# langtech-bsc/quantool

Measured on AMD Instinct MI355X. Metric: quantized weights/sec (GPTQ int4, Llama-3-8B, 512 calib samples), higher is better.
Workload: dtype f32

## Files before the change

quantool_amd/csrc/build.py:

```python
from __future__ import annotations

import hashlib
import os
import shutil
import subprocess
import sys
from concurrent.futures import ThreadPoolExecutor
from pathlib import Path

CSRC = Path(__file__).resolve().parent
PKG = CSRC.parent
LIB_DIR = PKG / "lib"
OBJ_DIR = CSRC / "_obj"
LIB_PATH = LIB_DIR / "libquantool_hip.so"

HIPCC_FLAGS = [
    "--offload-arch=gfx950",
    "-O3",
    "-fPIC",
    "-std=c++17",
    "-ffp-contract=off",
    "-fhip-fp32-correctly-rounded-divide-sqrt",
    "-fno-fast-math",
    "-Wall",
    "-Wno-unused-function",
    "-Rpass-analysis=kernel-resource-usage",
]

SCRATCH_OK: tuple = ()

HIPCC_FLAGS += os.environ.get("QT_EXTRA_HIPCC_FLAGS", "").split()


def _hipcc() -> str:
    for cand in (os.environ.get("HIPCC"), shutil.which("hipcc"), "/opt/rocm/bin/hipcc"):
        if cand and Path(cand).exists():
            return cand
    raise RuntimeError("hipcc not found (set HIPCC or install ROCm)")


def sources():
    return sorted(CSRC.glob("*.hip"))


def _stamp(src: Path) -> str:
    h = hashlib.sha1()
    h.update(src.read_bytes())
    for hdr in sorted(list(CSRC.glob("*.h")) + [PKG.parent / "include" / "quantool_amd.h"]):
        h.update(hdr.read_bytes())
    h.update(" ".join(HIPCC_FLAGS).encode())
    return h.hexdigest()


def _compile(src: Path) -> Path:
    obj = OBJ_DIR / (src.stem + ".o")
    stamp = OBJ_DIR / (src.stem + ".stamp")
    want = _stamp(src)
    if obj.exists() and stamp.exists() and stamp.read_text() == want:
        return obj
    cmd = [_hipcc(), *HIPCC_FLAGS, "-c", str(src), "-o", str(obj)]
    res = subprocess.run(cmd, capture_output=True, text=True)
    if res.returncode != 0:
        raise RuntimeError(f"hipcc failed for {src.name}:\n{res.stdout}\n{res.stderr}")
    rest = _resources(src, res.stderr)
    if rest.strip():
        sys.stderr.write(rest)
    stamp.write_text(want)
    return obj


def _resources(src: Path, stderr: str) -> str:
    import re

    kernels, cur, rest = [], None, []
    lines = stderr.splitlines()
    i = 0
    while i < len(lines):
        line = lines[i]
        m = re.search(r"remark:\s+(.*?) \[-Rpass-analysis=kernel-resource-usage\]", line)
        if m:
            kv = m.group(1).strip()
            if kv.startswith("Function Name:"):
                cur = {"name": kv.split(":", 1)[1].strip()}
                kernels.append(cur)
            elif cur is not None and ":" in kv:
                k, v = kv.rsplit(":", 1)
                cur[k.strip()] = v.strip()
            while i + 1 < len(lines) and re.match(r"^\s+\d* ?\|", lines[i + 1]):
                i += 1
        elif not re.match(r"^\d+ (warning|remark)s? generated", line.strip()) and "remarks generated" not in line:
            rest.append(line)
        i += 1
    rows = []
    for k in kernels:
        rows.append(f"{k['name']}\tvgpr {k.get('VGPRs', '?')}\tagpr {k.get('AGPRs', '?')}\tscratch "
                    f"{k.get('ScratchSize [bytes/lane]', '?')}\tvgpr_spill {k.get('VGPRs Spill', '?')}\tlds "
                    f"{k.get('LDS Size [bytes/block]', '?')}\twaves_per_simd {k.get('Occupancy [waves/SIMD]', '?')}")
    (OBJ_DIR / (src.stem + ".resources.txt")).write_text("\n".join(rows) + ("\n" if rows else ""))
    bad = [k["name"] for k in kernels
           if k.get("ScratchSize [bytes/lane]", "0") not in ("0", "?") and not any(ok in k["name"] for ok in SCRATCH_OK)]
    if bad:
        raise RuntimeError(f"{src.name}: kernel(s) with a private segment (scratch): {bad} -- see "
                           f"{OBJ_DIR / (src.stem + '.resources.txt')}; a by-value argument struct that is modified and "
                           "indexed at run time, or a register array indexed at run time, is the usual cause")
    return "\n".join(rest) + ("\n" if rest else "")


def audit_m0(src: Path) -> None:
    stamp = OBJ_DIR / (src.stem + ".m0audit")
    want = _stamp(src)
    if stamp.exists() and stamp.read_text() == want:
        return
    asm = OBJ_DIR / (src.stem + ".device.s")
    cmd = [_hipcc(), *[f for f in HIPCC_FLAGS if f != "-fPIC"], "--cuda-device-only", "-S", str(src), "-o", str(asm)]
    res = subprocess.run(cmd, capture_output=True, text=True)
    if res.returncode != 0:
        raise RuntimeError(f"hipcc -S failed for {src.name}:\n{res.stderr}")
    inside = False
    for n, line in enumerate(asm.read_text().splitlines(), 1):
        if ";;#ASMSTART" in line:
            inside = True
        elif ";;#ASMEND" in line:
            inside = False
        elif not inside and "m0" in line.split(";")[0].replace("_m0", ""):
            raise RuntimeError(f"{src.name}: compiler-generated use of M0 at {asm.name}:{n}: {line.strip()!r} -- "
                               "the LDS-DMA helpers must save/restore M0 again")
    audit_spills(src.name, asm.read_text())
    asm.unlink()
    stamp.write_text(want)


NO_SPILL_KERNELS = ("xtx_kernel", "xtx16_kernel", "gemm3_kernel", "sgemm_ring_kernel", "quantize_tokens_kernel",
                    "gemm_i8_kernel", "gemm_i8_ring_kernel", "gemm_i8_ring_moe_kernel", "gemm_i8_mid_kernel",
                    "gemm_i8_ring_w4_kernel", "gemm_i8_ring_w4_moe_kernel", "moe_gemm_i8_wide_kernel",
                    "moe_gemm_wq_wide_kernel")


def audit_spills(src_name: str, asm_text: str) -> None:
    name = None
    for line in asm_text.splitlines():
        t = line.strip()
        if t.startswith(".name:"):
            name = t.split(":", 1)[1].strip()
        elif name and t.startswith((".vgpr_spill_count:", ".private_segment_fixed_size:")):
            if int(t.split(":", 1)[1]) != 0 and any(k in name for k in NO_SPILL_KERNELS):
                raise RuntimeError(f"{src_name}: {name} spills ({t}) -- its schedule assumes every value stays in registers")


def build(verbose: bool = False) -> Path:
    OBJ_DIR.mkdir(exist_ok=True)
    LIB_DIR.mkdir(exist_ok=True)
    srcs = sources()
    with ThreadPoolExecutor(max_workers=min(8, len(srcs))) as ex:
        objs = list(ex.map(_compile, srcs))
    for name in ("xtx.hip", "gemm3_tn.hip", "sgemm_tn.hip", "qlinear.hip", "qlinear_ring.hip", "qlinear_ring_w4.hip"):
        audit_m0(CSRC / name)
    newest = max(o.stat().st_mtime for o in objs)
    if not LIB_PATH.exists() or LIB_PATH.stat().st_mtime < newest:
        cmd = [_hipcc(), "--offload-arch=gfx950", "-shared", "-fPIC", "-o", str(LIB_PATH), *map(str, objs)]
        res = subprocess.run(cmd, capture_output=True, text=True)
        if res.returncode != 0:
            raise RuntimeError(f"link failed:\n{res.stdout}\n{res.stderr}")
    if verbose:
        print(f"built {LIB_PATH}")
    return LIB_PATH


if __name__ == "__main__":
    build(verbose=True)
```

quantool_amd/csrc/cholesky.hip:

```cpp
#include <stdlib.h>
#include <string.h>

#include <map>
#include <tuple>
#include <vector>

#include "common.h"
#include "gemm3_tn.h"
#include "sgemm_tn.h"

namespace {

constexpr int NB = 128;
constexpr int NBO_MAX = 1024;
static int chol_block_env(const char* name) {
    const char* e = getenv(name);
    if (!e) return 0;
    int x = atoi(e) / 128 * 128;
    return x < 128 ? 128 : (x > NBO_MAX ? NBO_MAX : x);
}
struct G3Step {
    int n_items = 0, n_red = 0;
    size_t item_off = 0, red_off = 0;
};
struct CholG3Plan {
    bool any = false;
    std::vector<G3Step> fac, inv;
    char* blob = nullptr;
    size_t blob_bytes = 0;
    int max_slabs = 0;
};

static int chol_g3_min_chunks() {
    const char* on = getenv("QT_CHOL_G3");
    if (on && atoi(on) == 0) return 0;
    const char* e = getenv("QT_CHOL_G3_MIN_CHUNKS");
    const int x = e ? atoi(e) : 64;
    return x < 1 ? 1 : x;
}

static int chol_g3_target_items(int K) {
    const char* e = getenv("QT_G3_TARGET_ITEMS");
    if (e && atoi(e) > 0) return atoi(e);
    return K < 8192 ? 96 : 256;
}

static const CholG3Plan* chol_g3_plan(int K, int NBO, int NBI) {
    static std::mutex m;
    static std::map<std::tuple<int, int, int, int>, CholG3Plan*> plans;
    const int min_chunks = chol_g3_min_chunks();
    const int target_items = chol_g3_target_items(K);
    std::lock_guard<std::mutex> lock(m);
    const auto key = std::make_tuple(K, NBO, NBI, min_chunks * 1024 + target_items);
    auto it = plans.find(key);
    if (it != plans.end()) return it->second;
    CholG3Plan* pl = new CholG3Plan();
    std::vector<char> bytes;
    auto add = [&](int Tm, int Tn, int c_end, int tri) {
        G3Step st;
        if (min_chunks <= 0 || K % 8 != 0 || g3_row_chunks(Tm, Tn, c_end, tri) * G3_CHUNK_ROWS < (long)min_chunks * 128) return st;
        std::vector<G3Item> items;
        std::vector<G3Red> red;
        g3_plan_row(Tm, Tn, c_end, tri, items, red, target_items);
        st.n_items = (int)items.size();
        st.n_red = (int)red.size();
        st.item_off = qt_align_up(bytes.size(), 256);
        bytes.resize(st.item_off + items.size() * sizeof(G3Item));
        memcpy(bytes.data() + st.item_off, items.data(), items.size() * sizeof(G3Item));
        st.red_off = qt_align_up(bytes.size(), 256);
        bytes.resize(st.red_off + red.size() * sizeof(G3Red));
        if (!red.empty()) memcpy(bytes.data() + st.red_off, red.data(), red.size() * sizeof(G3Red));
        for (const G3Red& r : red) pl->max_slabs = pl->max_slabs > r.first + r.count ? pl->max_slabs : r.first + r.count;
        pl->any = true;
        return st;
    };
    for (int J0 = 0; J0 < K; J0 += NBO) {
        const int J1 = (K - J0 < NBO) ? K : J0 + NBO;
        pl->fac.push_back(J0 == 0 ? G3Step() : add((J1 - J0 + 255) / 256, (K - J0 + 255) / 256, J0 / G3_CHUNK_ROWS, 0));
    }
    for (int I0 = 0; I0 < K; I0 += NBI) {
        const int I1 = (K - I0 < NBI) ? K : I0 + NBI;
        pl->inv.push_back(I0 == 0 ? G3Step() : add((I1 - I0 + 255) / 256, (I0 + 255) / 256, I0 / G3_CHUNK_ROWS, 1));
    }
    if (pl->any) {
        pl->blob_bytes = qt_align_up(bytes.size(), 256);
        if (hipHostMalloc((void**)&pl->blob, pl->blob_bytes, hipHostMallocDefault) != hipSuccess) {
            pl->any = false;
            pl->blob = nullptr;
        } else {
            memcpy(pl->blob, bytes.data(), bytes.size());
        }
    }
    if (!pl->any) {
        pl->blob_bytes = 0;
        pl->max_slabs = 0;
        for (G3Step& st : pl->fac) st = G3Step();
        for (G3Step& st : pl->inv) st = G3Step();
    }
    plans[key] = pl;
    return pl;
}
static size_t chol_g3_ws_bytes(const CholG3Plan* pl, int K) {
    if (!pl->any) return 0;
    return 2 * qt_align_up((size_t)3 * K * K * 2, 256) + (size_t)pl->max_slabs * 256 * 256 * 4 + pl->blob_bytes + 256;
}

static const CholG3Plan* chol_blocks(int K, int& NBO, int& NBI) {
    const int eo = chol_block_env("QT_CHOL_NBO"), ei = chol_block_env("QT_CHOL_NBI");
    NBO = eo ? eo : 512;
    NBI = ei ? ei : 512;
    const CholG3Plan* pl = chol_g3_plan(K, NBO, NBI);
    if (pl->any) return pl;
    NBO = eo ? eo : 256;
    NBI = ei ? ei : 256;
    return chol_g3_plan(K, NBO, NBI);
}

constexpr int LDP = NB + 1;

constexpr int LDT = NB + 4;
constexpr int RD_STRIDE = NB * NB + 4 * 32 * 32;

#define QT_SEL4(kb, v0, v1, v2, v3) ((kb) == 0 ? (v0) : (kb) == 1 ? (v1) : (kb) == 2 ? (v2) : (v3))

constexpr int LDA = NB + 4;

__device__ __forceinline__ float readlane_f(float v, int lane) {
    return __int_as_float(__builtin_amdgcn_readlane(__float_as_int(v), lane));
}

__device__ __forceinline__ void mma32_tn(const float* A, int lda, const float* B, int ldb, f32x16& acc,
                                         int l31, int h, bool negate_a) {
#pragma unroll
    for (int kk = 0; kk < 16; ++kk) {
        float a = A[(2 * kk + h) * lda + l31];
        const float b = B[(2 * kk + h) * ldb + l31];
        if (negate_a) a = -a;
        acc = __builtin_amdgcn_mfma_f32_32x32x2f32(a, b, acc, 0, 0, 0);
    }
}

constexpr int POTF2_THREADS = 512, POTF2_WAVES = POTF2_THREADS / 64;
__global__ __launch_bounds__(POTF2_THREADS) void potf2_kernel(const float* P, int64_t ldp, int n,
                                                    float* Rout, int64_t ldr,
                                                    float* __restrict__ Rd, int32_t* info, int col0, int prio,
                                                    int64_t bsP, int64_t bsRd) {
    qt_set_chain_prio(prio);
    if (blockIdx.x) {
        P += (size_t)blockIdx.x * bsP;
        Rout += (size_t)blockIdx.x * bsP;
        Rd += (size_t)blockIdx.x * bsRd;
        info += blockIdx.x;
    }
    extern __shared__ __attribute__((aligned(16))) float sm[];
    float* As = sm;
    float* Xs = sm + NB * LDA;
    const int tid = threadIdx.x, lane = tid & 63;
    const int wave = __builtin_amdgcn_readfirstlane(tid >> 6);
    const int l31 = lane & 31, h = lane >> 5;

    if ((ldp & 3) == 0 && (n & 3) == 0 && (((uintptr_t)P) & 15) == 0) {
        constexpr int NV = NB * NB / 4 / POTF2_THREADS;
        f32x4 v[NV];
#pragma unroll
        for (int r = 0; r < NV; ++r) {
            const int e4 = tid + POTF2_THREADS * r;
            const int i = e4 >> 5, j = (e4 & 31) * 4;
            const int ic = i < n ? i : n - 1, jc = j < n ? j : n - 4;
            v[r] = *(const f32x4*)(P + (size_t)ic * ldp + jc);
        }
#pragma unroll
        for (int r = 0; r < NV; ++r) {
            const int e4 = tid + POTF2_THREADS * r;
            const int i = e4 >> 5, j = (e4 & 31) * 4;
            f32x4 x;
#pragma unroll
            for (int q = 0; q < 4; ++q) x[q] = (i < n && j + q < n) ? v[r][q] : (i == j + q ? 1.0f : 0.0f);
            *(f32x4*)(As + i * LDA + j) = x;
        }
    } else {
        for (int e = tid; e < NB * NB; e += POTF2_THREADS) {
            const int i = e / NB, j = e % NB;
            const int lo = i < j ? i : j, hi = i < j ? j : i;
            float v = (i == j) ? 1.0f : 0.0f;
            if (hi < n) v = P[(size_t)lo * ldp + hi];
            As[i * LDA + j] = v;
        }
    }
    __syncthreads();

    int bad = 0;
#pragma unroll 1
    for (int kb = 0; kb < 4; ++kb) {
        float* Akk = As + (32 * kb) * LDA + 32 * kb;
        if (wave == 0) {
            f32x16 c1, c2;
#pragma unroll
            for (int r = 0; r < 16; ++r) {
                const int i = (r & 3) + 8 * (r >> 2) + 4 * h;
                c1[r] = Akk[i * LDA + l31];
                c2[r] = (i == l31) ? 1.0f : 0.0f;
            }
#pragma unroll
            for (int c = 0; c < 32; ++c) {
                const int rc = (c & 3) + 4 * (c >> 3);
                const int hc = (c >> 2) & 1;
                float piv = readlane_f(c1[rc], c + 32 * hc);
                const bool isbad = !(piv > 0.0f);
                bad = (isbad && bad == 0 && 32 * kb + c < n) ? 32 * kb + c + 1 : bad;
                piv = isbad ? 1.0f : piv;
                float rs = __builtin_amdgcn_rsqf(piv);
                rs = rs * fmaf(-0.5f * piv * rs, rs, 1.5f);
                const bool mine = h == hc;
                const float rr = c1[rc] * rs, zz = c2[rc] * rs;
                c1[rc] = mine ? rr : c1[rc];
                c2[rc] = mine ? zz : c2[rc];
                if (c < 31) {
                    const float a = (mine && l31 > c) ? -rr : 0.0f;
                    const float b1 = (mine && l31 >= c) ? rr : 0.0f, b2 = mine ? zz : 0.0f;
                    c1 = __builtin_amdgcn_mfma_f32_32x32x2f32(a, b1, c1, 0, 0, 0);
                    c2 = __builtin_amdgcn_mfma_f32_32x32x2f32(a, b2, c2, 0, 0, 0);
                }
            }
#pragma unroll
            for (int r = 0; r < 16; ++r) {
                const int i = (r & 3) + 8 * (r >> 2) + 4 * h;
                Akk[i * LDA + l31] = (i <= l31) ? c1[r] : 0.0f;
                Xs[(kb * 32 + l31) * 32 + i] = (i >= l31) ? c2[r] : 0.0f;
            }
        }
        __syncthreads();
        if (kb == 3) break;
        for (int a = kb + 1 + wave; a < 4; a += POTF2_WAVES) {
            f32x16 acc;
#pragma unroll
            for (int r = 0; r < 16; ++r) acc[r] = 0.0f;
            float* Bt = As + (32 * kb) * LDA + 32 * a;
            mma32_tn(Xs + kb * 1024, 32, Bt, LDA, acc, l31, h, false);
#pragma unroll
            for (int r = 0; r < 16; ++r) Bt[((r & 3) + 8 * (r >> 2) + 4 * h) * LDA + l31] = acc[r];
        }
        __syncthreads();
        {
            int t = 0;
            for (int a = kb + 1; a < 4; ++a)
                for (int a2 = a; a2 < 4; ++a2, ++t) {
                    if ((t % POTF2_WAVES) != wave) continue;
                    float* Ct = As + (32 * a) * LDA + 32 * a2;
                    f32x16 acc;
#pragma unroll
                    for (int r = 0; r < 16; ++r) acc[r] = Ct[((r & 3) + 8 * (r >> 2) + 4 * h) * LDA + l31];
                    mma32_tn(As + (32 * kb) * LDA + 32 * a, LDA, As + (32 * kb) * LDA + 32 * a2, LDA, acc, l31, h,
                             true);
#pragma unroll
                    for (int r = 0; r < 16; ++r) Ct[((r & 3) + 8 * (r >> 2) + 4 * h) * LDA + l31] = acc[r];
                }
        }
        __syncthreads();
    }
    if (bad != 0 && tid == 0) atomicCAS(info, 0, col0 + bad);
    const bool vec_out = (ldr & 3) == 0 && (n & 3) == 0 && (((uintptr_t)Rout) & 15) == 0;
    for (int e4 = tid; e4 < NB * NB / 4; e4 += POTF2_THREADS) {
        const int i = e4 >> 5, j = (e4 & 31) * 4;
        f32x4 v = *(const f32x4*)(As + i * LDA + j);
#pragma unroll
        for (int q = 0; q < 4; ++q) v[q] = (j + q >= i) ? v[q] : 0.0f;
        *(f32x4*)(Rd + i * NB + j) = v;
        if (i < n && j + 3 >= i && j < n) {
            if (vec_out) {
                *(f32x4*)(Rout + (size_t)i * ldr + j) = v;
            } else {
#pragma unroll
                for (int q = 0; q < 4; ++q)
                    if (j + q >= i && j + q < n) Rout[(size_t)i * ldr + j + q] = v[q];
            }
        }
    }
    for (int e4 = tid; e4 < 4 * 32 * 32 / 4; e4 += POTF2_THREADS) *(f32x4*)(Rd + NB * NB + 4 * e4) = *(const f32x4*)(Xs + 4 * e4);
}

__global__ __launch_bounds__(256) void trsm_rt_kernel(const float* __restrict__ Rd, int n,
                                                      const float* B, int64_t ldb,
                                                      float* Z, int64_t ldz, int ncols, int prio, int64_t bsRd,
                                                      int64_t bsB) {
    qt_set_chain_prio(prio);
    if (blockIdx.y) {
        Rd += (size_t)blockIdx.y * bsRd;
        B += (size_t)blockIdx.y * bsB;
        Z += (size_t)blockIdx.y * bsB;
    }
    extern __shared__ __attribute__((aligned(16))) float Rs[];
    const int tid = threadIdx.x, lane = tid & 63, wave = tid >> 6;
    const float* D32 = Rs + NB * NB;
    const int l31 = lane & 31, h = lane >> 5;
    const int col = blockIdx.x * 128 + wave * 32 + l31;
    const bool cok = col < ncols;
    const int colc = cok ? col : ncols - 1;

    f32x16 acc[4];
#pragma unroll
    for (int a = 0; a < 4; ++a)
#pragma unroll
        for (int r = 0; r < 16; ++r) {
            const int row = 32 * a + (r & 3) + 8 * (r >> 2) + 4 * h;
            acc[a][r] = (row < n) ? B[(size_t)row * ldb + colc] : 0.0f;
        }
    {
        constexpr int NV = RD_STRIDE / 4 / 256;
        static_assert(NV * 4 * 256 == RD_STRIDE, "whole float4s per thread");
        f32x4 v[NV];
#pragma unroll
        for (int r = 0; r < NV; ++r) v[r] = ((const f32x4*)Rd)[tid + 256 * r];
#pragma unroll
        for (int r = 0; r < NV; ++r) ((f32x4*)Rs)[tid + 256 * r] = v[r];
    }
    __syncthreads();

#pragma unroll
    for (int b = 0; b < 4; ++b) {
        f32x16 zb;
#pragma unroll
        for (int r = 0; r < 16; ++r) zb[r] = 0.0f;
#pragma unroll
        for (int r = 0; r < 16; ++r) {
            const int k = (r & 3) + 8 * (r >> 2) + 4 * h;
            const float av = D32[(b * 32 + k) * 32 + l31];
            zb = __builtin_amdgcn_mfma_f32_32x32x2f32(av, acc[b][r], zb, 0, 0, 0);
        }
        acc[b] = zb;
#pragma unroll
        for (int a = b + 1; a < 4; ++a) {
#pragma unroll
            for (int r = 0; r < 16; ++r) {
                const int k = (r & 3) + 8 * (r >> 2) + 4 * h;
                const float av = -Rs[(32 * b + k) * NB + 32 * a + l31];
                acc[a] = __builtin_amdgcn_mfma_f32_32x32x2f32(av, zb[r], acc[a], 0, 0, 0);
            }
        }
    }
    if (cok) {
#pragma unroll
        for (int a = 0; a < 4; ++a)
#pragma unroll
            for (int r = 0; r < 16; ++r) {
                const int row = 32 * a + (r & 3) + 8 * (r >> 2) + 4 * h;
                if (row < n) Z[(size_t)row * ldz + col] = acc[a][r];
            }
    }
}

__global__ __launch_bounds__(128) void trinv_batched_kernel(const float* __restrict__ Rd_all, int K,
                                                            float* __restrict__ Dinv_all,
                                                            float* __restrict__ Y, int64_t ldy, int64_t bsW, int64_t bsY) {
    if (blockIdx.y) {
        Rd_all += (size_t)blockIdx.y * bsW;
        Dinv_all += (size_t)blockIdx.y * bsW;
        Y += (size_t)blockIdx.y * bsY;
    }
    extern __shared__ __attribute__((aligned(16))) float sm[];
    float* Rt = sm;
    float* Xs = sm + NB * LDT;
    const int b = blockIdx.x;
    const int n = (K - b * NB < NB) ? K - b * NB : NB;
    const float* Rd = Rd_all + (size_t)b * RD_STRIDE;
    const int j = threadIdx.x;
    for (int e = j; e < NB * NB; e += NB) {
        const int i = e / NB, c = e % NB;
        Rt[c * LDT + i] = Rd[e];
    }
    __syncthreads();
    float x0[32], x1[32], x2[32], x3[32];
#pragma unroll
    for (int r = 0; r < 32; ++r) {
        x0[r] = (r == j) ? 1.0f : 0.0f;
        x1[r] = (32 + r == j) ? 1.0f : 0.0f;
        x2[r] = (64 + r == j) ? 1.0f : 0.0f;
        x3[r] = (96 + r == j) ? 1.0f : 0.0f;
    }
#pragma unroll 1
    for (int pb = 3; pb >= 0; --pb) {
#pragma unroll
        for (int pp = 31; pp >= 0; --pp) {
            const int p = 32 * pb + pp;
            const float* rp = Rt + p * LDT;
            const float xp = QT_SEL4(pb, x0[pp], x1[pp], x2[pp], x3[pp]) / rp[p];
            if (pb == 0) x0[pp] = xp;
            if (pb == 1) x1[pp] = xp;
            if (pb == 2) x2[pp] = xp;
            if (pb == 3) x3[pp] = xp;
#define QT_XUPD(arr, a, r_to)                                                 \
    _Pragma("unroll") for (int r4 = 0; r4 < (r_to); r4 += 4) {                 \
        const f32x4 v4 = *(const f32x4*)(rp + 32 * (a) + r4);                 \
        _Pragma("unroll") for (int e = 0; e < 4; ++e)                         \
            if (r4 + e < (r_to)) arr[r4 + e] = fmaf(-v4[e], xp, arr[r4 + e]); \
    }
            if (pb == 0) { QT_XUPD(x0, 0, pp) } else { QT_XUPD(x0, 0, 32) }
            if (pb == 1) { QT_XUPD(x1, 1, pp) } else if (pb > 1) { QT_XUPD(x1, 1, 32) }
            if (pb == 2) { QT_XUPD(x2, 2, pp) } else if (pb > 2) { QT_XUPD(x2, 2, 32) }
            if (pb == 3) { QT_XUPD(x3, 3, pp) }
#undef QT_XUPD
        }
    }
#pragma unroll
    for (int r = 0; r < 32; ++r) {
        Xs[r * LDP + j] = x0[r];
        Xs[(32 + r) * LDP + j] = x1[r];
        Xs[(64 + r) * LDP + j] = x2[r];
        Xs[(96 + r) * LDP + j] = x3[r];
    }
    __syncthreads();
    float* Dinv = Dinv_all + (size_t)b * NB * NB;
    float* Yd = Y + (size_t)(b * NB) * ldy + b * NB;
    for (int e = j; e < NB * NB; e += NB) {
        const int i = e / NB, jj = e % NB;
        const bool in = (i < n && jj < n);
        Dinv[e] = (in && jj >= i) ? Xs[i * LDP + jj] : 0.0f;
        if (in) Yd[(size_t)i * ldy + jj] = (jj <= i) ? Xs[jj * LDP + i] : 0.0f;
    }
}

__global__ __launch_bounds__(256) void trinv_mfma_kernel(const float* __restrict__ Rd_all, int K,
                                                         float* __restrict__ Dinv_all,
                                                         float* __restrict__ Y, int64_t ldy, int64_t bsW, int64_t bsY) {
    if (blockIdx.y) {
        Rd_all += (size_t)blockIdx.y * bsW;
        Dinv_all += (size_t)blockIdx.y * bsW;
        Y += (size_t)blockIdx.y * bsY;
    }
    extern __shared__ __attribute__((aligned(16))) float Rs[];
    const int blk = blockIdx.x;
    const int n = (K - blk * NB < NB) ? K - blk * NB : NB;
    const float* Rd = Rd_all + (size_t)blk * RD_STRIDE;
    const int tid = threadIdx.x, lane = tid & 63, wave = tid >> 6;
    {
        constexpr int NV = RD_STRIDE / 4 / 256;
        f32x4 v[NV];
#pragma unroll
        for (int r = 0; r < NV; ++r) v[r] = ((const f32x4*)Rd)[tid + 256 * r];
#pragma unroll
        for (int r = 0; r < NV; ++r) ((f32x4*)Rs)[tid + 256 * r] = v[r];
    }
    const float* D32 = Rs + NB * NB;
    const int l31 = lane & 31, h = lane >> 5;
    const int col = wave * 32 + l31;

    f32x16 acc[4];
#pragma unroll
    for (int a = 0; a < 4; ++a)
#pragma unroll
        for (int r = 0; r < 16; ++r) {
            const int row = 32 * a + (r & 3) + 8 * (r >> 2) + 4 * h;
            acc[a][r] = (row == col) ? 1.0f : 0.0f;
        }
    __syncthreads();

#pragma unroll
    for (int b = 0; b < 4; ++b) {
        f32x16 zb;
#pragma unroll
        for (int r = 0; r < 16; ++r) zb[r] = 0.0f;
#pragma unroll
        for (int r = 0; r < 16; ++r) {
            const int k = (r & 3) + 8 * (r >> 2) + 4 * h;
            const float av = D32[(b * 32 + k) * 32 + l31];
            zb = __builtin_amdgcn_mfma_f32_32x32x2f32(av, acc[b][r], zb, 0, 0, 0);
        }
        acc[b] = zb;
#pragma unroll
        for (int a = b + 1; a < 4; ++a) {
#pragma unroll
            for (int r = 0; r < 16; ++r) {
                const int k = (r & 3) + 8 * (r >> 2) + 4 * h;
                const float av = -Rs[(32 * b + k) * NB + 32 * a + l31];
                acc[a] = __builtin_amdgcn_mfma_f32_32x32x2f32(av, zb[r], acc[a], 0, 0, 0);
            }
        }
    }
    float* Dinv = Dinv_all + (size_t)blk * NB * NB;
    float* Yd = Y + (size_t)(blk * NB) * ldy + blk * NB;
#pragma unroll
    for (int a = 0; a < 4; ++a)
#pragma unroll
        for (int r = 0; r < 16; ++r) {
            const int row = 32 * a + (r & 3) + 8 * (r >> 2) + 4 * h;
            const bool in = row < n && col < n;
            const float z = (in && row >= col) ? acc[a][r] : 0.0f;
            Dinv[col * NB + row] = z;
            if (in) Yd[(size_t)row * ldy + col] = z;
        }
}

__global__ __launch_bounds__(256) void transpose_lower_block_kernel(const float* __restrict__ Y, int64_t ldy, int w,
                                                                    float* __restrict__ XT, int ldx, int64_t bsY,
                                                                    int64_t bsXT) {
    if (blockIdx.z) {
        Y += (size_t)blockIdx.z * bsY;
        XT += (size_t)blockIdx.z * bsXT;
    }
    __shared__ float tile[32][33];
    const int bx = blockIdx.x * 32, by = blockIdx.y * 32;
    const int tx = threadIdx.x & 31, ty = threadIdx.x >> 5;
    for (int r = ty; r < 32; r += 8) {
        const int m = bx + r, k = by + tx;
        tile[r][tx] = (m < w && k < w && k <= m) ? Y[(size_t)m * ldy + k] : 0.0f;
    }
    __syncthreads();
    for (int r = ty; r < 32; r += 8) {
        const int k = by + r, m = bx + tx;
        if (k < w && m < w) XT[(size_t)k * ldx + m] = tile[tx][r];
    }
}

__global__ __launch_bounds__(256) void flat_reverse_lower_to_upper_kernel(float* __restrict__ U, int K, int64_t bsU) {
    U += (size_t)blockIdx.z * bsU;
    const int j = blockIdx.x * blockDim.x + threadIdx.x;
    const int i = blockIdx.y;
    if (j >= K || j < i) return;
    const size_t e = (size_t)i * K + j;
    const size_t pe = (size_t)(K - 1 - i) * K + (K - 1 - j);
    if (i == j) {
        if (e <= pe) {
            const float t = U[e];
            U[e] = U[pe];
            U[pe] = t;
        }
    } else {
        U[e] = U[pe];
        U[pe] = 0.0f;
    }
}

__global__ __launch_bounds__(256) void identity_if_failed_kernel(float* __restrict__ U, int K,
                                                                 const int32_t* __restrict__ info, int64_t bsU) {
    if (info[blockIdx.z] == 0) return;
    U += (size_t)blockIdx.z * bsU;
    for (int i = blockIdx.x; i < K; i += gridDim.x)
        for (int j = threadIdx.x; j < K; j += blockDim.x) U[(size_t)i * K + j] = (i == j) ? 1.0f : 0.0f;
}

__global__ __launch_bounds__(256) void chol_scales_kernel(const float* __restrict__ A, int64_t bsA, int K,
                                                          const float* __restrict__ min_eig_lb, int32_t* __restrict__ e,
                                                          int32_t* __restrict__ info) {
    __shared__ float red[256];
    const int b = blockIdx.x, nprob = gridDim.x;
    const float* Ab = A + (size_t)b * bsA;
    float m = 0.0f;
    for (int i = threadIdx.x; i < K; i += 256) m = fmaxf(m, Ab[(size_t)i * K + i]);
    red[threadIdx.x] = m;
    __syncthreads();
    for (int s = 128; s > 0; s >>= 1) {
        if ((int)threadIdx.x < s) red[threadIdx.x] = fmaxf(red[threadIdx.x], red[threadIdx.x + s]);
        __syncthreads();
    }
    if (threadIdx.x == 0) {
        auto clampe = [](float t) { return (int)fminf(fmaxf(t, (float)-G3_E_MAX), (float)G3_E_MAX); };
        const float d = red[0], lb = min_eig_lb[b];
        e[b] = (d > 0.0f && d < 3.0e38f) ? clampe(3.0f - ceilf(0.5f * log2f(d))) : 0;
        if (lb > 0.0f && lb < 3.0e38f) {
            e[nprob + b] = clampe(3.0f - ceilf(-0.5f * log2f(lb)));
        } else {
            e[nprob + b] = 0;
            info[b] = K + 1;
        }
    }
}

}

static size_t chol_problem_ws_bytes(int K, const CholG3Plan* g3) {
    const size_t nb = (K + NB - 1) / NB;
    const size_t split = (size_t)2048 * NB * NB * 4 + (size_t)NBO_MAX * K * 4;
    size_t n = (size_t)NB * K * 4 + (size_t)NBO_MAX * K * 4 + (size_t)NBO_MAX * NBO_MAX * 4 + nb * (NB * NB + RD_STRIDE) * 4 + split + 256;
    if (g3->any) n += 2 * qt_align_up((size_t)3 * K * K * 2, 256) + (size_t)g3->max_slabs * 256 * 256 * 4 + 256;
    return qt_align_up(n, 256);
}

extern "C" size_t qt_cholesky_inverse_upper_batched_workspace_bytes(int K, int n_problems) {
    if (K <= 0 || n_problems <= 0) return 0;
    int nbo_, nbi_;
    const CholG3Plan* g3 = chol_blocks(K, nbo_, nbi_);
    return (size_t)n_problems * chol_problem_ws_bytes(K, g3) + g3->blob_bytes + 512;
}

extern "C" size_t qt_cholesky_inverse_upper_workspace_bytes(int K) {
    return qt_cholesky_inverse_upper_batched_workspace_bytes(K, 1);
}

static int chol_run(float* A, int64_t strideA, int K, float* U, int64_t strideU, int32_t* info, int nprob, void* workspace,
                    size_t workspace_bytes, hipStream_t stream, const float* min_eig_lb = nullptr) {
    bool f16x2 = min_eig_lb != nullptr;
    if (const char* e = getenv("QT_CHOL_PLANES")) {
        if (strcmp(e, "bf16x3") == 0) f16x2 = false;
        else if (strcmp(e, "f16x2") == 0) {
            QT_CHECK_ARG(min_eig_lb, "qt_cholesky_inverse_upper: QT_CHOL_PLANES=f16x2 needs a bound on lambda_min (the _bounded entry points)");
        } else {
            QT_CHECK_ARG(false, "qt_cholesky_inverse_upper: QT_CHOL_PLANES=%s (bf16x3 | f16x2)", e);
        }
    }
    const size_t need = qt_cholesky_inverse_upper_batched_workspace_bytes(K, nprob);
    if (!workspace || workspace_bytes < need) {
        qt_set_error("qt_cholesky_inverse_upper: workspace %zu < required %zu", workspace_bytes, need);
        return QT_ERR_WORKSPACE;
    }
    const int nblk = (K + NB - 1) / NB;
    char* ws = (char*)qt_align_up((size_t)workspace, 256);
    int NBO, NBI;
    const CholG3Plan* g3 = chol_blocks(K, NBO, NBI);
    const size_t prob_bytes = chol_problem_ws_bytes(K, g3);
    const int64_t sW = (int64_t)(prob_bytes / 4);
    const int64_t sA = nprob > 1 ? strideA : 0, sU = nprob > 1 ? strideU : 0;
    float* T = (float*)ws;
    float* TI = T + (size_t)NB * K;
    float* XT = TI + (size_t)NBO_MAX * K;
    float* Rd = XT + (size_t)NBO_MAX * NBO_MAX;
    float* Dinv = Rd + (size_t)nblk * RD_STRIDE;
    float* split_ws = Dinv + (size_t)nblk * NB * NB;
    const size_t split_ws_bytes = (size_t)2048 * NB * NB * 4 + (size_t)NBO_MAX * K * 4;
    unsigned short *Rpl = nullptr, *Ypl = nullptr;
    float* g3_slabs = nullptr;
    char* g3_tab = nullptr;
    const int64_t plane_stride = (int64_t)K * K;
    if (g3->any) {
        char* q = (char*)qt_align_up((size_t)((char*)split_ws + split_ws_bytes), 256);
        Rpl = (unsigned short*)q;
        q += qt_align_up((size_t)3 * K * K * 2, 256);
        Ypl = (unsigned short*)q;
        q += qt_align_up((size_t)3 * K * K * 2, 256);
        g3_slabs = (float*)q;
        g3_tab = (char*)qt_align_up((size_t)(ws + (size_t)nprob * prob_bytes), 256);
        QT_HIP(hipMemcpyAsync(g3_tab, g3->blob, g3->blob_bytes, hipMemcpyHostToDevice, stream));
    }
    f16x2 = f16x2 && g3->any;
    int32_t* eR = f16x2 ? (int32_t*)(Rpl + 2 * plane_stride) : nullptr;
    int32_t* eY = f16x2 ? eR + nprob : nullptr;
    static_assert(2 * SG_MAX_BATCH * sizeof(int32_t) <= (size_t)NB * NB * 2, "the exponents fit the smallest third plane");
    auto g3_row = [&](const G3Step& st, const unsigned short* Bplanes, int col_a0, int col_b0, int M, int N, float* C,
                      int64_t bsC, int mode) -> int {
        G3Args a;
        a.Apl = Rpl;
        a.Bpl = Bplanes;
        a.plane_stride = plane_stride;
        a.ld = K;
        a.rowA0 = a.rowB0 = 0;
        a.colA0 = col_a0;
        a.colB0 = col_b0;
        a.colmax = K;
        a.M = M;
        a.N = N;
        a.C = C;
        a.ldc = K;
        a.mode = mode;
        a.slabs = g3_slabs;
        a.items = (const G3Item*)(g3_tab + st.item_off);
        a.n_items = st.n_items;
        a.red = (const G3Red*)(g3_tab + st.red_off);
        a.n_red = st.n_red;
        a.batch = nprob;
        a.bsApl = a.bsBpl = sW * 2;
        a.bsC = bsC;
        a.bsSlabs = sW;
        if (f16x2) {
            a.planes = G3_F16X2;
            a.eA = eR;
            a.eB = Bplanes == Rpl ? eR : eY;
        }
        return qt_gemm3_launch(a, stream);
    };
    auto sgemm = [&](SgemmArgs& g, int64_t bsA_, int64_t bsB_, int64_t bsC_) -> int {
        g.batch = nprob;
        g.bsA = bsA_;
        g.bsB = bsB_;
        g.bsCin = g.bsCout = bsC_;
        g.bs_split = sW;
        return qt_sgemm_tn(g, stream);
    };
    float* Y = U;
    const int64_t sY = sU;
    const size_t inv_lds = (size_t)(NB * LDT + NB * LDP) * sizeof(float);
    const size_t potf2_lds = (size_t)(NB * LDA + 4 * 32 * 32) * sizeof(float);
    static QtOncePerDevice lds_attr;
    QT_HIP(lds_attr.run([&] {
        hipError_t e = hipFuncSetAttribute((const void*)potf2_kernel, hipFuncAttributeMaxDynamicSharedMemorySize,
                                           (int)potf2_lds);
        if (e == hipSuccess)
            e = hipFuncSetAttribute((const void*)trsm_rt_kernel, hipFuncAttributeMaxDynamicSharedMemorySize,
                                    (int)(RD_STRIDE * sizeof(float)));
        if (e == hipSuccess)
            e = hipFuncSetAttribute((const void*)trinv_batched_kernel, hipFuncAttributeMaxDynamicSharedMemorySize,
                                    (int)inv_lds);
        if (e == hipSuccess)
            e = hipFuncSetAttribute((const void*)trinv_mfma_kernel, hipFuncAttributeMaxDynamicSharedMemorySize,
                                    (int)(RD_STRIDE * sizeof(float)));
        return e;
    }));
    QT_HIP(hipMemsetAsync(info, 0, sizeof(int32_t) * nprob, stream));
    const int prio = qt_chain_prio();
    if (f16x2) {
        hipLaunchKernelGGL(chol_scales_kernel, dim3(nprob), dim3(256), 0, stream, (const float*)A, sA, K, min_eig_lb, eR, info);
        QT_LAUNCH_CHECK();
    }

    for (int J0 = 0, Jb = 0; J0 < K; J0 += NBO, ++Jb) {
        const int J1 = (K - J0 < NBO) ? K : J0 + NBO;
        if (g3->any && J0 > 0) {
            const G3Step& st = g3->fac[Jb];
            float* C = A + (size_t)J0 * K + J0;
            if (st.n_items > 0) {
                int rc = g3_row(st, Rpl, J0, J0, J1 - J0, K - J0, C, sA, G3_SUB);
                if (rc) return rc;
            } else {
                SgemmArgs g;
                g.A = A + J0; g.lda = K;
                g.B = A + J0; g.ldb = K;
                g.Cin = C; g.ldcin = K;
                g.Cout = C; g.ldcout = K;
                g.M = J1 - J0; g.N = K - J0; g.kdim = J0; g.k_mode = SG_K_FULL; g.mode = SG_MODE_SUB;
                g.split_ws = split_ws; g.split_ws_bytes = split_ws_bytes;
                int rc = sgemm(g, sA, sA, sA);
                if (rc) return rc;
            }
        }
        for (int j0 = J0; j0 < J1; j0 += NB) {
            const int j = j0 / NB, nbj = (K - j0 < NB) ? K - j0 : NB;
            float* Ajj = A + (size_t)j0 * K + j0;
            if (j0 > J0) {
                SgemmArgs g;
                g.A = A + (size_t)J0 * K + j0; g.lda = K;
                g.B = A + (size_t)J0 * K + j0; g.ldb = K;
                g.Cin = Ajj; g.ldcin = K;
                g.Cout = Ajj; g.ldcout = K;
                g.M = nbj; g.N = K - j0; g.kdim = j0 - J0; g.k_mode = SG_K_FULL; g.mode = SG_MODE_SUB;
                int rc = sgemm(g, sA, sA, sA);
                if (rc) return rc;
            }
            hipLaunchKernelGGL(potf2_kernel, dim3(nprob), dim3(POTF2_THREADS), potf2_lds, stream, (const float*)Ajj, (int64_t)K, nbj,
                               Ajj, (int64_t)K, Rd + (size_t)j * RD_STRIDE, info, j0, prio, sA, sW);
            QT_LAUNCH_CHECK();
            const int rest = K - j0 - nbj;
            if (rest > 0) {
                hipLaunchKernelGGL(trsm_rt_kernel, dim3((rest + 127) / 128, nprob), dim3(256), RD_STRIDE * sizeof(float),
                                   stream, (const float*)(Rd + (size_t)j * RD_STRIDE), nbj, (const float*)(Ajj + nbj),
                                   (int64_t)K, Ajj + nbj, (int64_t)K, rest, prio, sW, sA);
                QT_LAUNCH_CHECK();
            }
        }
        const int rem = K - J1;
        if (g3->any) {
            if (rem > 0) {
                int rc = f16x2 ? qt_split2h_launch(A + (size_t)J0 * K + J0, K, J1 - J0, K - J0, Rpl + (size_t)J0 * K + J0, K,
                                                   plane_stride, 0, 0, 0, eR, stream, nprob, sA, sW * 2)
                               : qt_split3_launch(A + (size_t)J0 * K + J0, K, J1 - J0, K - J0, Rpl + (size_t)J0 * K + J0, K,
                                                  plane_stride, 0, 0, 0, stream, nprob, sA, sW * 2);
                if (rc) return rc;
            }
        } else if (rem > 0) {
            SgemmArgs g;
            g.A = A + (size_t)J0 * K + J1; g.lda = K;
            g.B = A + (size_t)J0 * K + J1; g.ldb = K;
            g.Cin = A + (size_t)J1 * K + J1; g.ldcin = K;
            g.Cout = A + (size_t)J1 * K + J1; g.ldcout = K;
            g.M = rem; g.N = rem; g.kdim = J1 - J0; g.k_mode = SG_K_FULL; g.mode = SG_MODE_SUB;
            g.upper_only = 1;
            int rc = sgemm(g, sA, sA, sA);
            if (rc) return rc;
        }
    }
    {
        const char* e = getenv("QT_CHOL_TRINV");
        if (e && strcmp(e, "div") == 0)
            hipLaunchKernelGGL(trinv_batched_kernel, dim3(nblk, nprob), dim3(NB), inv_lds, stream, (const float*)Rd, K, Dinv, Y,
                               (int64_t)K, sW, sY);
        else
            hipLaunchKernelGGL(trinv_mfma_kernel, dim3(nblk, nprob), dim3(256), RD_STRIDE * sizeof(float), stream,
                               (const float*)Rd, K, Dinv, Y, (int64_t)K, sW, sY);
    }
    QT_LAUNCH_CHECK();
    for (int I0 = 0, Ib = 0; I0 < K; I0 += NBI, ++Ib) {
        const int I1 = (K - I0 < NBI) ? K : I0 + NBI;
        const int Wi = I1 - I0;
        for (int i0 = I0 + NB; i0 < I1; i0 += NB) {
            const int i = i0 / NB, nbi = (K - i0 < NB) ? K - i0 : NB;
            SgemmArgs g;
            g.A = A + (size_t)I0 * K + i0; g.lda = K;
            g.B = Y + (size_t)I0 * K + I0; g.ldb = K;
            g.Cin = nullptr; g.ldcin = 0;
            g.Cout = T; g.ldcout = K;
            g.M = nbi; g.N = i0 - I0; g.kdim = i0 - I0; g.k_mode = SG_K_FROM_N0; g.mode = SG_MODE_SET;
            int rc = sgemm(g, sA, sY, sW);
            if (rc) return rc;
            SgemmArgs t;
            t.A = Dinv + (size_t)i * NB * NB; t.lda = NB;
            t.B = T; t.ldb = K;
            t.Cin = nullptr; t.ldcin = 0;
            t.Cout = Y + (size_t)i0 * K + I0; t.ldcout = K;
            t.M = nbi; t.N = i0 - I0; t.kdim = nbi; t.k_mode = SG_K_FULL; t.mode = SG_MODE_NEG;
            rc = sgemm(t, sW, sW, sY);
            if (rc) return rc;
        }
        auto split_row = [&]() -> int {
            if (!g3->any || I1 >= K) return QT_OK;
            if (f16x2)
                return qt_split2h_launch(Y + (size_t)I0 * K, K, Wi, I1, Ypl + (size_t)I0 * K, K, plane_stride, 1, I0, 0, eY,
                                         stream, nprob, sY, sW * 2);
            return qt_split3_launch(Y + (size_t)I0 * K, K, Wi, I1, Ypl + (size_t)I0 * K, K, plane_stride, 1, I0, 0, stream,
                                    nprob, sY, sW * 2);
        };
        if (I0 == 0) {
            int rc0 = split_row();
            if (rc0) return rc0;
            continue;
        }
        int rc;
        if (g3->any && g3->inv[Ib].n_items > 0) {
            rc = g3_row(g3->inv[Ib], Ypl, I0, 0, Wi, I0, TI, sW, G3_SET);
        } else {
            SgemmArgs g;
            g.A = A + I0; g.lda = K;
            g.B = Y; g.ldb = K;
            g.Cin = nullptr; g.ldcin = 0;
            g.Cout = TI; g.ldcout = K;
            g.M = Wi; g.N = I0; g.kdim = I0; g.k_mode = SG_K_FROM_N0; g.mode = SG_MODE_SET;
            g.split_ws = split_ws; g.split_ws_bytes = split_ws_bytes;
            rc = sgemm(g, sA, sY, sW);
        }
        if (rc) return rc;
        hipLaunchKernelGGL(transpose_lower_block_kernel, dim3((Wi + 31) / 32, (Wi + 31) / 32, nprob), dim3(256), 0, stream,
                           (const float*)(Y + (size_t)I0 * K + I0), (int64_t)K, Wi, XT, NBO_MAX, sY, sW);
        QT_LAUNCH_CHECK();
        SgemmArgs t;
        t.A = XT; t.lda = NBO_MAX;
        t.B = TI; t.ldb = K;
        t.Cin = nullptr; t.ldcin = 0;
        t.Cout = Y + (size_t)I0 * K; t.ldcout = K;
        t.M = Wi; t.N = I0; t.kdim = Wi; t.k_mode = SG_K_FULL; t.mode = SG_MODE_NEG;
        rc = sgemm(t, sW, sW, sY);
        if (rc) return rc;
        rc = split_row();
        if (rc) return rc;
    }
    hipLaunchKernelGGL(flat_reverse_lower_to_upper_kernel, dim3((K + 255) / 256, K, nprob), dim3(256), 0, stream, U, K, sU);
    QT_LAUNCH_CHECK();
    hipLaunchKernelGGL(identity_if_failed_kernel, dim3(K < 1024 ? K : 1024, 1, nprob), dim3(256), 0, stream, U, K,
                       (const int32_t*)info, sU);
    QT_LAUNCH_CHECK();
    return QT_OK;
}

extern "C" int qt_cholesky_inverse_upper(float* A, int K, float* U, int32_t* info, void* workspace,
                                         size_t workspace_bytes, qt_stream_t stream_) {
    QT_CHECK_ARG(K > 0 && A && U && info, "qt_cholesky_inverse_upper: bad arguments");
    return chol_run(A, 0, K, U, 0, info, 1, workspace, workspace_bytes, (hipStream_t)stream_);
}

extern "C" int qt_cholesky_inverse_upper_batched(float* A, int64_t strideA, int K, float* U, int64_t strideU, int32_t* info,
                                                 int n_problems, void* workspace, size_t workspace_bytes,
                                                 qt_stream_t stream_) {
    QT_CHECK_ARG(K > 0 && A && U && info && n_problems >= 1 && n_problems <= SG_MAX_BATCH,
                 "qt_cholesky_inverse_upper_batched: bad arguments (1 <= n_problems <= %d)", SG_MAX_BATCH);
    QT_CHECK_ARG(n_problems == 1 || (strideA >= (int64_t)K * K && strideU >= (int64_t)K * K && strideA % 4 == 0 && strideU % 4 == 0),
                 "qt_cholesky_inverse_upper_batched: strides must be multiples of 4 elements and >= K*K");
    return chol_run(A, strideA, K, U, strideU, info, n_problems, workspace, workspace_bytes, (hipStream_t)stream_);
}

extern "C" int qt_cholesky_inverse_upper_bounded(float* A, int K, float* U, int32_t* info, const float* min_eig_lb,
                                                 void* workspace, size_t workspace_bytes, qt_stream_t stream_) {
    QT_CHECK_ARG(K > 0 && A && U && info && min_eig_lb, "qt_cholesky_inverse_upper_bounded: bad arguments");
    return chol_run(A, 0, K, U, 0, info, 1, workspace, workspace_bytes, (hipStream_t)stream_, min_eig_lb);
}

extern "C" int qt_cholesky_inverse_upper_batched_bounded(float* A, int64_t strideA, int K, float* U, int64_t strideU,
                                                         int32_t* info, int n_problems, const float* min_eig_lb,
                                                         void* workspace, size_t workspace_bytes, qt_stream_t stream_) {
    QT_CHECK_ARG(K > 0 && A && U && info && min_eig_lb && n_problems >= 1 && n_problems <= SG_MAX_BATCH,
                 "qt_cholesky_inverse_upper_batched_bounded: bad arguments (1 <= n_problems <= %d)", SG_MAX_BATCH);
    QT_CHECK_ARG(n_problems == 1 || (strideA >= (int64_t)K * K && strideU >= (int64_t)K * K && strideA % 4 == 0 && strideU % 4 == 0),
                 "qt_cholesky_inverse_upper_batched_bounded: strides must be multiples of 4 elements and >= K*K");
    return chol_run(A, strideA, K, U, strideU, info, n_problems, workspace, workspace_bytes, (hipStream_t)stream_, min_eig_lb);
}
```

Baseline: 3.198 billion.

## Fuse diagonal-block triangular inverse sweep into one MFMA kernel per block

Replaces the per-128-row loop of paired sgemm launches (T = A*Y, then Y = -Dinv*T) inside each NBI diagonal block with a single kernel. One workgroup handles each NBI block and steps through the sub-blocks, staging T in LDS and using 32x32x2 f32 MFMA with register prefetch. This removes many small kernel launches and the round trips of T through global memory. The cost is that each NBI block is processed serially by one 512-thread workgroup, which limits parallelism, and the build script now fails if this kernel spills registers.

```diff
diff --git a/quantool_amd/csrc/build.py b/quantool_amd/csrc/build.py
--- a/quantool_amd/csrc/build.py
+++ b/quantool_amd/csrc/build.py
@@ -103,6 +103,11 @@
         raise RuntimeError(f"{src.name}: kernel(s) with a private segment (scratch): {bad} -- see "
                            f"{OBJ_DIR / (src.stem + '.resources.txt')}; a by-value argument struct that is modified and "
                            "indexed at run time, or a register array indexed at run time, is the usual cause")
+    spilled = [k["name"] for k in kernels if any(n in k["name"] for n in NO_SPILL_KERNELS)
+               and k.get("VGPRs Spill", "0") not in ("0", "?")]
+    if spilled:
+        raise RuntimeError(f"{src.name}: {spilled} spill(s) -- the schedule assumes every value stays in registers; see "
+                           f"{OBJ_DIR / (src.stem + '.resources.txt')}")
     return "\n".join(rest) + ("\n" if rest else "")
 
 
@@ -133,7 +138,7 @@
 NO_SPILL_KERNELS = ("xtx_kernel", "xtx16_kernel", "gemm3_kernel", "sgemm_ring_kernel", "quantize_tokens_kernel",
                     "gemm_i8_kernel", "gemm_i8_ring_kernel", "gemm_i8_ring_moe_kernel", "gemm_i8_mid_kernel",
                     "gemm_i8_ring_w4_kernel", "gemm_i8_ring_w4_moe_kernel", "moe_gemm_i8_wide_kernel",
-                    "moe_gemm_wq_wide_kernel")
+                    "moe_gemm_wq_wide_kernel", "trinv_block_kernel")
 
 
 def audit_spills(src_name: str, asm_text: str) -> None:
diff --git a/quantool_amd/csrc/cholesky.hip b/quantool_amd/csrc/cholesky.hip
--- a/quantool_amd/csrc/cholesky.hip
+++ b/quantool_amd/csrc/cholesky.hip
@@ -488,6 +488,117 @@
             Dinv[col * NB + row] = z;
             if (in) Yd[(size_t)row * ldy + col] = z;
         }
+}
+
+constexpr int YB_THREADS = 512;
+constexpr int YB_LD = 128;
+__global__ __launch_bounds__(YB_THREADS) void trinv_block_kernel(const float* A, float* Y,
+                                                                 const float* __restrict__ Dinv_all, int K, int NBI,
+                                                                 int64_t bsA, int64_t bsY, int64_t bsW) {
+    __shared__ __attribute__((aligned(16))) float Ts[NB * YB_LD];
+    if (blockIdx.y) {
+        A += (size_t)blockIdx.y * bsA;
+        Y += (size_t)blockIdx.y * bsY;
+        Dinv_all += (size_t)blockIdx.y * bsW;
+    }
+    const int I0 = blockIdx.x * NBI;
+    const int I1 = (K - I0 < NBI) ? K : I0 + NBI;
+    const int nst = (I1 - I0 + NB - 1) / NB - 1;
+    const int tid = threadIdx.x, lane = tid & 63;
+    const int wave = __builtin_amdgcn_readfirstlane(tid >> 6);
+    const int mt = wave >> 1, cl = wave & 1;
+    const int h = lane >> 5, l31 = lane & 31;
+    const size_t ld = (size_t)K;
+
+    for (int j = 0; j < nst; ++j) {
+        const int n0 = NB * j + 64 * cl;
+        for (int s = j + 1; s <= nst; ++s) {
+            const int i0 = I0 + NB * s;
+            const int nbi = (K - i0 < NB) ? K - i0 : NB;
+            const bool wave_on = 32 * mt < nbi;
+            const int m = 32 * mt + l31;
+            const bool m_ok = m < nbi;
+            f32x16 acc0, acc1;
+#pragma unroll
+            for (int r = 0; r < 16; ++r) acc0[r] = acc1[r] = 0.0f;
+
+            if (wave_on) {
+                const int ke = NB * s;
+                const float* ap = A + (size_t)(I0 + h) * ld + i0 + (m_ok ? m : nbi - 1);
+                const float* bp = Y + (size_t)(I0 + h) * ld + I0 + n0 + l31;
+                float a[8], b0[8], b1[8], an[8], b0n[8], b1n[8];
+#pragma unroll
+                for (int u = 0; u < 8; ++u) {
+                    a[u] = ap[(size_t)(n0 + 2 * u) * ld];
+                    b0[u] = bp[(size_t)(n0 + 2 * u) * ld];
+                    b1[u] = bp[(size_t)(n0 + 2 * u) * ld + 32];
+                }
+                for (int k = n0; k < ke; k += 16) {
+                    const int kn = k + 16 < ke ? k + 16 : k;
+#pragma unroll
+                    for (int u = 0; u < 8; ++u) {
+                        an[u] = ap[(size_t)(kn + 2 * u) * ld];
+                        b0n[u] = bp[(size_t)(kn + 2 * u) * ld];
+                        b1n[u] = bp[(size_t)(kn + 2 * u) * ld + 32];
+                    }
+#pragma unroll
+                    for (int u = 0; u < 8; ++u) {
+                        const float av = m_ok ? a[u] : 0.0f;
+                        acc0 = __builtin_amdgcn_mfma_f32_32x32x2f32(av, b0[u], acc0, 0, 0, 0);
+                        acc1 = __builtin_amdgcn_mfma_f32_32x32x2f32(av, b1[u], acc1, 0, 0, 0);
+                    }
+#pragma unroll
+                    for (int u = 0; u < 8; ++u) {
+                        a[u] = an[u];
+                        b0[u] = b0n[u];
+                        b1[u] = b1n[u];
+                    }
+                }
+            }
+#pragma unroll
+            for (int r = 0; r < 16; ++r) {
+                const int row = 32 * mt + (r & 3) + 8 * (r >> 2) + 4 * h;
+                const bool in = row < nbi;
+                Ts[row * YB_LD + 64 * cl + l31] = in ? acc0[r] : 0.0f;
+                Ts[row * YB_LD + 64 * cl + 32 + l31] = in ? acc1[r] : 0.0f;
+            }
+            __syncthreads();
+
+            if (wave_on) {
+                const int ke = (nbi + 15) / 16 * 16;
+                const float* dp = Dinv_all + (size_t)(i0 / NB) * NB * NB + h * NB + m;
+                const float* tp = Ts + h * YB_LD + 64 * cl + l31;
+#pragma unroll
+                for (int r = 0; r < 16; ++r) acc0[r] = acc1[r] = 0.0f;
+                float a[8], an[8];
+#pragma unroll
+                for (int u = 0; u < 8; ++u) a[u] = dp[2 * u * NB];
+                for (int k = 0; k < ke; k += 16) {
+                    const int kn = k + 16 < ke ? k + 16 : k;
+#pragma unroll
+                    for (int u = 0; u < 8; ++u) an[u] = dp[(kn + 2 * u) * NB];
+#pragma unroll
+                    for (int u = 0; u < 8; ++u) {
+                        const float b0 = tp[(k + 2 * u) * YB_LD], b1 = tp[(k + 2 * u) * YB_LD + 32];
+                        acc0 = __builtin_amdgcn_mfma_f32_32x32x2f32(a[u], b0, acc0, 0, 0, 0);
+                        acc1 = __builtin_amdgcn_mfma_f32_32x32x2f32(a[u], b1, acc1, 0, 0, 0);
+                    }
+#pragma unroll
+                    for (int u = 0; u < 8; ++u) a[u] = an[u];
+                }
+                float* yp = Y + (size_t)i0 * ld + I0 + n0 + l31;
+#pragma unroll
+                for (int r = 0; r < 16; ++r) {
+                    const int row = 32 * mt + (r & 3) + 8 * (r >> 2) + 4 * h;
+                    if (row < nbi) {
+                        yp[(size_t)row * ld] = -acc0[r];
+                        yp[(size_t)row * ld + 32] = -acc1[r];
+                    }
+                }
+            }
+            __syncthreads();
+        }
+    }
 }
 
 __global__ __launch_bounds__(256) void transpose_lower_block_kernel(const float* __restrict__ Y, int64_t ldy, int w,
@@ -775,10 +886,17 @@
                                (const float*)Rd, K, Dinv, Y, (int64_t)K, sW, sY);
     }
     QT_LAUNCH_CHECK();
+    bool yii_loop = false;
+    if (const char* e = getenv("QT_CHOL_YII")) yii_loop = strcmp(e, "loop") == 0;
+    if (!yii_loop && NBI > NB && K > NB) {
+        hipLaunchKernelGGL(trinv_block_kernel, dim3((K + NBI - 1) / NBI, nprob), dim3(YB_THREADS), 0, stream, (const float*)A, Y,
+                           (const float*)Dinv, K, NBI, sA, sY, sW);
+        QT_LAUNCH_CHECK();
+    }
     for (int I0 = 0, Ib = 0; I0 < K; I0 += NBI, ++Ib) {
         const int I1 = (K - I0 < NBI) ? K : I0 + NBI;
         const int Wi = I1 - I0;
-        for (int i0 = I0 + NB; i0 < I1; i0 += NB) {
+        for (int i0 = I0 + NB; yii_loop && i0 < I1; i0 += NB) {
             const int i = i0 / NB, nbi = (K - i0 < NB) ? K - i0 : NB;
             SgemmArgs g;
             g.A = A + (size_t)I0 * K + i0; g.lda = K;
```

Result: no change. 3.230 billion (median of 6 runs) (+1.0%).
